# facebookresearch/spdl

Hardware: AMD Instinct MI355X
Metric: images/sec device-resident JPEG→RGB224, 1/2/4/8×MI355X; % HBM roofline (higher is better)
Workload: dtype u8; 1 GPU; configs[1]: synthetic 480x640 q90 4:2:0 baseline JPEG resident in HBM -> RGB 224x224 u8 (scale bicubic decrease + centred pad, rgb24); global_batch=256, per_gpu_batch=256, distinct_images=32, lanes=4, hw_queues=4, entropy_threads=256, entropy_piece_bytes=131072

## Files before the change

### spdl_amd/csrc/hj_common.h

```cpp
#pragma once
#include <stddef.h>
#include <stdint.h>

#ifndef HJ_HD
#define HJ_HD __host__ __device__
#endif

namespace hj {

constexpr int kMaxComp = 4;

enum { kColorGray = 0, kColorYcbcr, kColorRgb, kColorCmyk, kColorYcck, kColorYcbcrk };
inline HJ_HD bool frame_color(int ncomp, const int32_t* h, const int32_t* v, const int* ids,
                              int adobe, int32_t* color) {
  bool all11 = true;
  for (int c = 0; c < ncomp; c++) all11 = all11 && h[c] == 1 && v[c] == 1;
  if (ncomp == 1) {
    *color = kColorGray;
  } else if (ncomp == 3) {
    const bool rgb = adobe == 0 || (ids[0] == 'R' && ids[1] == 'G' && ids[2] == 'B');
    if (rgb && !all11) return false;
    *color = rgb ? kColorRgb : kColorYcbcr;
  } else {
    if (!all11) return false;
// ... 159 lines not shown
};
inline HJ_HD IdctDivMod idct_divmod(uint32_t n, uint32_t d, uint32_t magic) {
  uint32_t q = (uint32_t)(((uint64_t)n * magic) >> 32);
  uint32_t r = n - q * d;
  if (r >= d) {
    q += 1;
    r -= d;
  }
  return {q, r};
}
struct IdctBlockPos {
  int c, bx, by;
};
inline HJ_HD IdctBlockPos idct_block_pos(const ImageInfo& in, uint32_t j) {
  const IdctDivMod m = idct_divmod(j, (uint32_t)in.bpm, in.bpm_magic);
  const IdctDivMod p = idct_divmod(m.q, (uint32_t)in.mcux, in.mcux_magic);
  const int b = (int)m.r, c = in.mcu_comp[b];
  if (in.ncomp == 1) return {c, (int)p.r, (int)p.q};
  return {c, (int)p.r * in.comp_h[c] + in.mcu_dx[b], (int)p.q * in.comp_v[c] + in.mcu_dy[b]};
}

inline HJ_HD uint32_t idct_region_block(const ImageInfo& in, int mx0, int my0, int mw,
                                        uint32_t mw_magic, uint32_t l) {
  const IdctDivMod m = idct_divmod(l, (uint32_t)in.bpm, in.bpm_magic);
  const IdctDivMod p = idct_divmod(m.q, (uint32_t)mw, mw_magic);
  return ((uint32_t)(my0 + (int)p.q) * (uint32_t)in.mcux + (uint32_t)(mx0 + (int)p.r)) *
             (uint32_t)in.bpm + m.r;
}

constexpr int kDsChunk = 4096;
constexpr int kIdctThreads = 256;
constexpr int kHsRows = 16;
struct DsChunk {
  int32_t keep, rst, term;
  int32_t keep_pre, rst_pre;
  int32_t pad_[3];
};

struct SwsCsc {
  int32_t crv, cbu, cgu, cgv;
  int32_t y_coeff, y_offset, v2r, v2g, u2g, u2b;
};

#ifndef HJ_ABLATIONS
#define HJ_ABLATIONS 0
#endif
enum Ablate : int32_t {
  kAblSwsHpass = 0x100,
  kAblSwsVpass = 0x200,
  kAblSwsStore = 0x400,
  kAblIdctNone = 0x800,
  kAblEntWrite = 0x1000,
  kAblEntSync = 0x2000,
  kAblEntList = 0x4000,
  kAblEntDc = 0x8000,
  kAblEntDesc = 0x80000,
  kAblEntropy = kAblEntWrite | kAblEntSync | kAblEntList | kAblEntDc | kAblEntDesc,
  kAblNoMultiscan = 0x10000,
  kAblNoIdct = 0x20000,
  kAblNoOutput = 0x40000,
};

struct BatchParams {
  int32_t n;
  int32_t pix_fmt, dtype, idct;
  int32_t resize, filter;
  int32_t out_w, out_h;
  int32_t sub_bits;
  int32_t debug_mask;
// ... 31 lines not shown
```

### spdl_amd/csrc/hj_destuff.h

```cpp
#pragma once
#include <cstdint>

#ifndef HJ_HD
#define HJ_HD __host__ __device__
#endif

namespace hj {

HJ_HD inline int ds_ctz(uint32_t v) {
#if defined(__HIP_DEVICE_COMPILE__)
  return __ffs((int)v) - 1;
#else
  return __builtin_ctz(v);
#endif
}
HJ_HD inline int ds_top(uint32_t v) {
#if defined(__HIP_DEVICE_COMPILE__)
  return 31 - __clz((int)v);
#else
  return 31 - __builtin_clz(v);
#endif
}
HJ_HD inline int ds_popc(uint32_t v) {
#if defined(__HIP_DEVICE_COMPILE__)
// ... 140 lines not shown
    }
  }
}

HJ_HD inline void ds_compact_begin(uint32_t (&w)[4], uint32_t keep, uint32_t& drop) {
#pragma unroll
  for (int i = 0; i < 4; i++) {
    const uint32_t m = (((keep >> (4 * i)) & 15u) * 0x204081u) & 0x01010101u;
    w[i] &= ds_perm(0u, 0u, 0x0C0C0C0Cu + m);
  }
  drop = keep ? ~keep & ((1u << ds_top(keep)) - 1u) & ~((1u << ds_ctz(keep)) - 1u) : 0u;
}

HJ_HD inline void ds_compact_step(uint32_t (&w)[4], uint32_t& drop) {
  const int p = ds_ctz(drop | 0x10000u);
  drop = (drop >> 1) & (0xFFFFFFFFu << p);
  const uint32_t up = 0xFFFF0000u >> (16 - p);
#pragma unroll
  for (int i = 0; i < 4; i++) {
    const uint32_t inc = (((up >> (4 * i)) & 15u) * 0x204081u) & 0x01010101u;
    w[i] = ds_perm(i < 3 ? w[i + 1] : 0u, w[i], 0x03020100u + inc);
  }
}

HJ_HD inline void ds_shift_words(const uint32_t (&w)[4], uint32_t s, uint32_t (&x)[5]) {
  const uint32_t sel = 0x07060504u - ds_perm(0u, s, 0u);
  x[0] = ds_perm(w[0], 0u, sel);
  x[1] = ds_perm(w[1], w[0], sel);
  x[2] = ds_perm(w[2], w[1], sel);
  x[3] = ds_perm(w[3], w[2], sel);
  x[4] = ds_perm(0u, w[3], sel);
}

}
```

### spdl_amd/csrc/hj_kernels.hip

```cpp
#include <hip/hip_fp16.h>
#include <hip/hip_runtime.h>

#include "hj_common.h"
#include "hj_destuff.h"
#include "hj_idct.h"
#include "hj_launch.h"
#include "hj_sws_tile.h"
#include "hj_upsample.h"

namespace hj {

__device__ __forceinline__ uint32_t rfl(uint32_t v) { return __builtin_amdgcn_readfirstlane(v); }


struct ParseScratch {
  ImageInfo info;
  uint16_t qt[4][64];
  uint8_t bits[8][17];
  uint8_t vals[8][256];
  int32_t have[8];
  int32_t qhave[4];
  int32_t maxcode[8][18];
  int32_t valoff[8][17];
  int32_t dqt_off[4], dqt_pq[4];
// ... 177 lines not shown
          for (int y = 0; y < in.comp_v[c]; y++)
            for (int x = 0; x < in.comp_h[c]; x++) {
              if (b >= kMaxBpm) return kErrUnsupported;
              in.mcu_comp[b] = c;
              in.mcu_dx[b] = x;
              in.mcu_dy[b] = y;
              b++;
            }
        }
        in.bpm = b;
      }
      in.nblocks = in.mcux * in.mcuy * in.bpm;
      in.bpm_magic = idct_div_magic((uint32_t)in.bpm);
      in.mcux_magic = idct_div_magic((uint32_t)in.mcux);
      return kOk;
    }
  }
}

__global__ void __launch_bounds__(256, 8) parse_kernel(const uint8_t* __restrict__ bytes,
                                                    const ImageDesc* __restrict__ host_desc,
                                                    ImageDesc* __restrict__ desc,
                                                    ImageInfo* __restrict__ infos,
                                                    HuffTable* __restrict__ luts,
                                                    const uint4* __restrict__ host_tables,
                                                    uint4* __restrict__ tables, int64_t ntab16,
                                                    const uint32_t* __restrict__ host_work,
                                                    uint32_t* __restrict__ work, int nwork,
                                                    uint64_t* __restrict__ chain,
                                                    uint32_t* __restrict__ ds_map,
                                                    uint32_t* __restrict__ idct_map,
                                                    uint32_t* __restrict__ hs_map,
                                                    uint32_t* __restrict__ sws_map,
                                                    const int ndesc) {
  __shared__ ParseScratch s;
  __shared__ int st;
  __shared__ __attribute__((aligned(16))) uint8_t hdr[kHdrBytes];
  const int img = blockIdx.x, tid = threadIdx.x;
#if HJ_PARSE_PROF
  int64_t pt[8];
  int npt = 0;
  pt[npt++] = wall_clock64();
#define HJ_PT() (pt[npt++] = wall_clock64())
#else
#define HJ_PT() ((void)0)
#endif
  __shared__ __attribute__((aligned(16))) ImageDesc sdd;
  {
    static_assert(sizeof(ImageDesc) % 8 == 0, "descriptor copied in 8-byte words");
    const uint64_t* src = reinterpret_cast<const uint64_t*>((host_desc ? host_desc : desc) + img);
    uint64_t* dst = reinterpret_cast<uint64_t*>(desc + img);
    uint64_t* sdst = reinterpret_cast<uint64_t*>(&sdd);
    for (int i = tid; i < (int)(sizeof(ImageDesc) / 8); i += blockDim.x) {
      const uint64_t v = src[i];
      if (host_desc) dst[i] = v;
      sdst[i] = v;
    }
  }
  if (host_desc) {
    for (int64_t i = (int64_t)img * blockDim.x + tid; i < ntab16;
         i += (int64_t)gridDim.x * blockDim.x)
      tables[i] = host_tables[i];
    for (int i = img * blockDim.x + tid; i < nwork; i += gridDim.x * blockDim.x)
      work[i] = host_work[i];
  }
  for (int v = (int)gridDim.x + img; v < ndesc; v += (int)gridDim.x) {
    const ImageDesc* sv = (host_desc ? host_desc : desc) + v;
    if (host_desc) {
      const uint64_t* src = reinterpret_cast<const uint64_t*>(sv);
      uint64_t* dst = reinterpret_cast<uint64_t*>(desc + v);
      for (int i = tid; i < (int)(sizeof(ImageDesc) / 8); i += blockDim.x) dst[i] = src[i];
    }
    const int hs0 = sv->hs_wg0, hsn = sv->hs_wgs, sw0 = sv->sws_wg0,
              swn = sv->sws_bands * sv->sws_chunks;
    for (int i = tid; i < hsn; i += blockDim.x) hs_map[hs0 + i] = (uint32_t)v;
    for (int i = tid; i < swn; i += blockDim.x) sws_map[sw0 + i] = (uint32_t)v;
  }
  __syncthreads();
  const ImageDesc& dd = sdd;
  for (int i = tid; i < dd.ds_cap; i += blockDim.x) ds_map[dd.ds_wg0 + i] = (uint32_t)img;
  for (int i = tid; i < (dd.idct_blocks + kIdctThreads - 1) / kIdctThreads; i += blockDim.x)
    idct_map[dd.idct_wg0 + i] = (uint32_t)img;
  for (int i = tid; i < dd.hs_wgs; i += blockDim.x) hs_map[dd.hs_wg0 + i] = (uint32_t)img;
  for (int i = tid; i < dd.sws_bands * dd.sws_chunks; i += blockDim.x)
    sws_map[dd.sws_wg0 + i] = (uint32_t)img;
  if (img == 0 && tid == 0) chain[0] = 0ull;
  if (dd.pieces > 1)
    for (int i = tid; i < dd.pieces * kChainGranules; i += blockDim.x)
      chain[kChainHead + dd.chain_off + i] = 0ull;
  {
    int* z = reinterpret_cast<int*>(&s);
    for (int i = tid; i < (int)(sizeof(ParseScratch) / 4); i += blockDim.x) z[i] = 0;
  }
  const int nh = (int)min(dd.in_size, (int64_t)kHdrBytes) & ~15;
  for (int i = tid; i < nh / 16; i += blockDim.x)
    reinterpret_cast<uint4*>(hdr)[i] = reinterpret_cast<const uint4*>(bytes + dd.in_off)[i];
  __syncthreads();
  HJ_PT();
  if (tid == 0) {
    const Bytes file{bytes + dd.in_off, (lds_u8*)hdr, nh};
    int rc = parse_headers(file, (int)dd.in_size, s);
    if (rc == kOk) {
      if (s.info.width != dd.width || s.info.height != dd.height || s.info.ncomp != dd.ncomp ||
          s.info.nblocks != dd.nblocks || s.info.color != dd.color)
        rc = kErrBadHeader;
      for (int c = 0; c < s.info.ncomp && rc == kOk; c++)
        if (s.info.comp_h[c] != dd.h_samp[c] || s.info.comp_v[c] != dd.v_samp[c])
          rc = kErrBadHeader;
      if (rc == kOk && s.info.ri > 0 &&
          (s.info.mcux * s.info.mcuy + s.info.ri - 1) / s.info.ri > dd.seg_cap)
        rc = kErrBadRestart;
    }
    if (rc == kOk && dd.refuse) rc = dd.refuse;
// ... 84 lines not shown
    tab_nsub[t] = nsub;
  }
  __syncthreads();
  if (tid == 0) {
    int ns = 0, seen = 0, subs = 0, slow = 0;
    for (int c = 0; c < s.info.ncomp; c++)
      for (int k = 0; k < 2; k++) {
        const int slot = k == 0 ? s.info.dc_tab[c] : 4 + s.info.ac_tab[c];
        if (!(seen & (1 << slot))) {
          ns++;
          subs += tab_nsub[slot];
          slow |= (tab_slow >> slot) & 1;
          slow |= tab_nsub[slot] > (kSubShare >> kSubBits);
        }
        seen |= 1 << slot;
      }
    s.info.ent_wide = !(ns <= 4 && (subs << kSubBits) <= kSubPool && !slow);
  }
  __syncthreads();
  HJ_PT();
#if HJ_PARSE_PROF
  if (tid == 0)
    for (int i = 1; i < npt && i < 8; i++) s.info.sdiag[39 + i] = (int32_t)(pt[i] - pt[0]);
#endif
  static_assert(sizeof(ImageInfo) % 4 == 0, "ImageInfo copied in words");
  {
    const uint32_t* src = reinterpret_cast<const uint32_t*>(&s.info);
    uint32_t* dst = reinterpret_cast<uint32_t*>(infos + img);
    for (int i = tid; i < (int)(sizeof(ImageInfo) / 4); i += blockDim.x) dst[i] = src[i];
  }
}


__global__ void __launch_bounds__(256) lut_kernel(const uint8_t* __restrict__ bytes,
                                                  const ImageDesc* __restrict__ desc,
                                                  ImageInfo* __restrict__ infos,
                                                  HuffTable* __restrict__ luts) {
  __shared__ int first, same, maxcode[18], valoff[17];
  __shared__ uint8_t bits[17], vals[256];
  const int t = blockIdx.x, img = blockIdx.y, tid = threadIdx.x;
  const ImageInfo& in = infos[img];
  if (in.status != kOk || in.multiscan || in.tab_n[t] == 0) return;
  const uint32_t h = in.tab_hash[t];
  const int n = in.tab_n[t];
  const uint8_t* d = bytes + desc[img].in_off + in.tab_off[t];
  if (tid == 0) first = img;
  __syncthreads();
  for (int j = tid; j < img; j += blockDim.x) {
    const ImageInfo& o = infos[j];
    if (o.status == kOk && !o.multiscan && o.tab_n[t] == n && o.tab_hash[t] == h)
      atomicMin(&first, j);
  }
  __syncthreads();
  const int j = first;
  if (j < img) {
    if (tid == 0) same = 1;
    __syncthreads();
    const uint8_t* e = bytes + desc[j].in_off + infos[j].tab_off[t];
    for (int k = tid; k < 16 + n; k += blockDim.x)
      if (d[k] != e[k]) same = 0;
    __syncthreads();
    if (same) {
      if (tid == 0) infos[img].lut_ref[t] = j * 8 + t;
      return;
    }
  }
  if (tid < 16) bits[tid + 1] = d[tid];
  for (int k = tid; k < 256; k += blockDim.x) vals[k] = k < n ? d[16 + k] : 0;
  __syncthreads();
  if (tid == 0) {
    int code = 0, k = 0;
    for (int l = 1; l <= 16; l++) {
      if (bits[l]) {
        valoff[l] = k - code;
        code += bits[l];
        k += bits[l];
        maxcode[l] = code - 1;
      } else {
        maxcode[l] = -1;
        valoff[l] = 0;
      }
      code <<= 1;
    }
    maxcode[17] = 0x7FFFFFFF;
// ... 22 lines not shown
          if (sz) {
            const int raw = (int)((w16 >> (16 - l - sz)) & ((1u << sz) - 1));
            v = raw < (1 << (sz - 1)) ? raw - ((1 << sz) - 1) : raw;
          }
          return hj_entry(kKindFull, l + sz, sym, is_dc, v);
        }
        return hj_entry(kKindCode, l, sym, is_dc, 0);
      }
    }
    return 0u;
  };
  for (int idx = tid; idx < kLutSize; idx += blockDim.x) {
    uint32_t e = entry16((uint32_t)idx << kSubBits, kLutBits, kLutBits);
    if (e == 0u && idx >= p_lo && idx <= p_hi)
      e = sub_ok ? ((kKindSub << 5) | ((uint32_t)(idx - p_lo) << kEntHiShift)) : 0u;
    T.lut[idx] = e ? e : 1u;
  }
  if (sub_ok)
    for (int i = tid; i < nsub << kSubBits; i += blockDim.x)
      T.sub[i] = max(entry16(((uint32_t)(p_lo + (i >> kSubBits)) << kSubBits) |
                                 (uint32_t)(i & ((1 << kSubBits) - 1)),
                             16, 16),
                     1u);
  if (tid == 0) {
    T.nsub = sub_ok ? nsub : 0;
    T.long_slow = sub_ok ? 0 : 1;
    T.sub_lo = sub_ok ? p_lo : 0;
  }
  if (tid < 18) T.maxcode[tid] = maxcode[tid];
  if (tid < 17) T.valoff[tid] = valoff[tid];
  for (int i = tid; i < 256; i += blockDim.x) T.vals[i] = vals[i];
}


constexpr int kDsThreads = 256;
constexpr int kDsPer = kDsChunk / kDsThreads;

__device__ __forceinline__ int wave_incl_scan(int v) {
  const int lane = threadIdx.x & 63;
#pragma unroll
  for (int d = 1; d < 64; d <<= 1) {
    const int u = __shfl_up(v, d, 64);
    if (lane >= d) v += u;
  }
  return v;
}

__device__ __forceinline__ void wg_scan2(int a, int b, int& ea, int& eb, int& ta, int& tb,
                                        int* sh ) {
  const int lane = threadIdx.x & 63, wid = threadIdx.x >> 6;
  const int ia = wave_incl_scan(a), ib = wave_incl_scan(b);
  if (lane == 63) {
    sh[wid] = ia;
    sh[4 + wid] = ib;
  }
  __syncthreads();
  ea = ia - a;
  eb = ib - b;
  ta = tb = 0;
#pragma unroll
  for (int w = 0; w < 4; w++) {
    if (w < wid) {
      ea += sh[w];
      eb += sh[4 + w];
    }
    ta += sh[w];
    tb += sh[4 + w];
  }
}

__device__ __forceinline__ int wave_incl_scan_dpp(int v) {
  v += __builtin_amdgcn_update_dpp(0, v, 0x111, 0xF, 0xF, false);
  v += __builtin_amdgcn_update_dpp(0, v, 0x112, 0xF, 0xF, false);
  v += __builtin_amdgcn_update_dpp(0, v, 0x114, 0xF, 0xF, false);
  v += __builtin_amdgcn_update_dpp(0, v, 0x118, 0xF, 0xF, false);
  v += __builtin_amdgcn_update_dpp(0, v, 0x142, 0xA, 0xF, false);
  v += __builtin_amdgcn_update_dpp(0, v, 0x143, 0xC, 0xF, false);
  return v;
}

__device__ __forceinline__ void wg_scan1(int v, int& ex, int& tot, int* sh ) {
  const int lane = threadIdx.x & 63, wid = threadIdx.x >> 6;
  const int iv = wave_incl_scan_dpp(v);
  if (lane == 63) sh[wid] = iv;
  __syncthreads();
  ex = iv - v;
  tot = 0;
#pragma unroll
  for (int w = 0; w < 4; w++) {
    if (w < wid) ex += sh[w];
    tot += sh[w];
  }
}

__device__ __forceinline__ void ds_load(const uint8_t* __restrict__ d, int size, int j0,
                                        uint32_t (&w)[4], uint32_t& prev, uint32_t& next) {
  prev = ds_prev_byte(d, size, j0);
  if (j0 + 16 <= size) {
    const uint4 q = *reinterpret_cast<const uint4*>(d + j0);
    w[0] = q.x;
    w[1] = q.y;
    w[2] = q.z;
    w[3] = q.w;
  } else {
    ds_load_bytes(d, size, j0, w);
  }
  next = ds_next_byte(d, size, j0);
}

constexpr int kDsStageWords = (16 + 16 + kDsChunk + 32) / 4;

__device__ __forceinline__ void stage_to_global(uint8_t* __restrict__ dst, const uint32_t* stage,
                                                int n, int tid) {
  const int a = (int)((uintptr_t)dst & 15);
  const uint8_t* src = reinterpret_cast<const uint8_t*>(stage) + 16 + a;
  const int head = min(n, (16 - a) & 15);
  if (tid < head) dst[tid] = src[tid];
  const int nv = (n - head) >> 4;
  const uint4* s4 = reinterpret_cast<const uint4*>(src + head);
  uint4* d4 = reinterpret_cast<uint4*>(dst + head);
  for (int i = tid; i < nv; i += kDsThreads) d4[i] = s4[i];
  const int t0 = head + 16 * nv;
  if (t0 + tid < n) dst[t0 + tid] = src[t0 + tid];
}

__global__ void __launch_bounds__(kDsThreads) destuff_count_kernel(
    const uint8_t* __restrict__ bytes, const ImageDesc* __restrict__ desc,
    const ImageInfo* __restrict__ infos, DsChunk* __restrict__ chunks,
    const uint32_t* __restrict__ ds_map) {
  __shared__ int shsum, shterm;
  const bool flat = ds_map != nullptr;
  const int img = flat ? (int)ds_map[blockIdx.x] : (int)blockIdx.y;
  const int k = flat ? (int)blockIdx.x - desc[img].ds_wg0 : (int)blockIdx.x, tid = threadIdx.x;
  if (infos[img].status != kOk || infos[img].multiscan) return;
  const ImageDesc& dd = desc[img];
  const int size = (int)dd.in_size, start = infos[img].scan_start;
  const int cbase = (start & ~15) + k * kDsChunk;
  if (cbase >= size || k >= dd.ds_cap) return;
  if (tid == 0) {
    shsum = 0;
    shterm = 0x7FFFFFFF;
  }
  __syncthreads();
  const uint8_t* d = bytes + dd.in_off;
  const int j0 = cbase + tid * kDsPer;
  uint32_t w[4], prev, next;
  ds_load(d, size, j0, w, prev, next);
  uint32_t slow;
  int cnt = ds_count_words(w, prev, next, j0, start, size, slow);
  if (slow) {
    uint32_t rst;
    int term;
    ds_resolve(d, size, j0, slow, rst, term);
    cnt += __popc(rst) << 16;
    if (term != 0x7FFFFFFF) atomicMin(&shterm, term);
  }
  const int wsum = wave_incl_scan_dpp(cnt);
  if ((tid & 63) == 63) atomicAdd(&shsum, wsum);
  __syncthreads();
  if (tid == 0) {
    DsChunk& c = chunks[dd.ds_off + k];
    c.keep = shsum & 0xFFFF;
    c.rst = shsum >> 16;
    c.term = shterm;
  }
}

__global__ void __launch_bounds__(kDsThreads) destuff_prefix_kernel(
    const ImageDesc* __restrict__ desc, ImageInfo* __restrict__ infos,
    DsChunk* __restrict__ chunks) {
  __shared__ int sh[8];
  __shared__ int shterm;
  const int img = blockIdx.x, tid = threadIdx.x;
  if (infos[img].status != kOk || infos[img].multiscan) return;
  const ImageDesc& dd = desc[img];
  const int size = (int)dd.in_size, start = infos[img].scan_start;
  const int base = start & ~15;
  const int nch = min(dd.ds_cap, (size - base + kDsChunk - 1) / kDsChunk);
  if (tid == 0) shterm = 0x7FFFFFFF;
  __syncthreads();
  for (int k = tid; k < nch; k += kDsThreads) atomicMin(&shterm, chunks[dd.ds_off + k].term);
  __syncthreads();
  const int end = min(shterm, size);
  int ck = 0, cr = 0;
  for (int k0 = 0; k0 < nch; k0 += kDsThreads) {
    const int k = k0 + tid;
    const bool v = k < nch && base + k * kDsChunk < end;
    const int kk = v ? chunks[dd.ds_off + k].keep : 0, rr = v ? chunks[dd.ds_off + k].rst : 0;
    int ek, er, tk, tr;
    wg_scan2(kk, rr, ek, er, tk, tr, sh);
    if (k < nch) {
      chunks[dd.ds_off + k].keep_pre = ck + ek;
      chunks[dd.ds_off + k].rst_pre = cr + er;
    }
    ck += tk;
    cr += tr;
    __syncthreads();
  }
  if (tid == 0) infos[img].scan_end = end;
}

__global__ void __launch_bounds__(kDsThreads) destuff_write_kernel(
    const uint8_t* __restrict__ bytes, const ImageDesc* __restrict__ desc,
    ImageInfo* __restrict__ infos, const DsChunk* __restrict__ chunks, uint8_t* __restrict__ clean,
    uint32_t* __restrict__ segs, const uint32_t* __restrict__ ds_map) {
  __shared__ int sh[4];
  __shared__ __attribute__((aligned(16))) uint32_t stage[kDsStageWords];
  const bool flat = ds_map != nullptr;
  const int img = flat ? (int)ds_map[blockIdx.x] : (int)blockIdx.y;
  const int k = flat ? (int)blockIdx.x - desc[img].ds_wg0 : (int)blockIdx.x, tid = threadIdx.x;
  if (infos[img].status != kOk || infos[img].multiscan) return;
  const ImageDesc& dd = desc[img];
  const int size = (int)dd.in_size, start = infos[img].scan_start, end = infos[img].scan_end;
  const int base = start & ~15;
  const int cbase = base + k * kDsChunk;
  const int last = (max(end - 1, start) - base) / kDsChunk;
  if (k > last || k >= dd.ds_cap) return;
  for (int i = tid; i < kDsStageWords / 4; i += kDsThreads)
    reinterpret_cast<uint4*>(stage)[i] = make_uint4(0, 0, 0, 0);
  const uint8_t* d = bytes + dd.in_off;
  const int j0 = cbase + tid * kDsPer;
  uint32_t w[4], prev, next;
  ds_load(d, size, j0, w, prev, next);
  const DsMasks m = ds_classify_words(w, prev, next, j0, start, end);
  const uint32_t keep = m.keep;
  uint32_t rst = 0;
  if (m.slow) {
    int term;
    ds_resolve(d, size, j0, m.slow, rst, term);
  }
  int ex, tot;
  wg_scan1((int)(__popc(rst) << 16 | __popc(keep)), ex, tot, sh);
  const int ek = ex & 0xFFFF, er = ex >> 16, tk = tot & 0xFFFF, tr = tot >> 16;
  const DsChunk& c = chunks[dd.ds_off + k];
  uint32_t* sg = segs + dd.seg_off;
  if (rst) {
    int r = c.rst_pre + er;
    bool overflow = false;
    for (uint32_t q = rst; q; q &= q - 1) {
      const int i = ds_ctz(q);
      r++;
      if (r < dd.seg_cap) sg[r] = (uint32_t)(c.keep_pre + ek + __popc(keep & ((1u << i) - 1u)));
      else overflow = true;
    }
    if (overflow) infos[img].status = kErrBadRestart;
  }
  uint8_t* out = clean + dd.in_off + c.keep_pre;
  uint32_t drop;
  ds_compact_begin(w, keep, drop);
  while (__any(drop != 0u)) ds_compact_step(w, drop);
  if (keep) {
    const int p = 16 + (int)((uintptr_t)out & 15) + ek - ds_ctz(keep);
    uint32_t x[5];
    ds_shift_words(w, (uint32_t)(p & 3), x);
    uint32_t* q = stage + (p >> 2);
#pragma unroll
    for (int i = 0; i < 5; i++) atomicOr(q + i, x[i]);
  }
  __syncthreads();
  stage_to_global(out, stage, tk, tid);
  if (k == last) {
    const int clen = c.keep_pre + tk;
    if (tid < 64) out[tk + tid] = 0;
    if (tid == 0) {
      infos[img].clean_len = clen;
      infos[img].nseg = min(c.rst_pre + tr + 1, dd.seg_cap);
      sg[0] = 0;
    }
  }
}


constexpr int kMaxTabs = 2 * kMaxComp;
__constant__ uint8_t kSlotOrder[64] = {
    0,  4,  8,  16, 12, 1,  5,  9,  20, 24, 32, 28, 17, 13, 2,  6,  10, 21, 25, 36, 40, 48,
    44, 33, 29, 18, 14, 3,  7,  11, 22, 26, 37, 41, 52, 56, 60, 49, 45, 34, 30, 19, 15, 23,
    27, 38, 42, 53, 57, 61, 50, 46, 35, 31, 39, 43, 54, 58, 62, 51, 47, 55, 59, 63};
constexpr int kWinWords = 12;

template <int NT, int NTAB>
struct EntShared {
  static constexpr int kTabs = NTAB;
  uint32_t lut[NTAB][kLutSize];
  uint32_t sub[kSubPool];
  int32_t maxcode[NTAB][18];
  int32_t valoff[NTAB][17];
  uint8_t vals[NTAB][256];
  uint32_t run_pos[NT];
  uint32_t run_zb[NT];
  uint32_t qdc[kMaxComp];
  union {
    uint32_t win[kWinWords][NT];
    struct {
      int32_t scan_flag[NT];
      int32_t scan_v[NT][kMaxComp];
      int32_t red[NT];
    } sc;
  };
  int32_t flag;
// ... 387 lines not shown
    done = (bad && past_a) || stop || (trunc && past_b);
    rc = (bad && !past_a) ? kErrBadHuffman : ((trunc && !past_b) ? kErrTruncated : kOk);
    const bool bend = zn >= 64u;
    if (bend && !stop && o.open) close_block(o, nb - 1);
    const uint32_t bsn = hot_next(m, d.bs);
    d.z = bend ? 0u : zn;
    d.bs = bend ? bsn : d.bs;
  }
  if (o.open && d.z != 0u) close_block(o, nb - 1);
  hot_flip(m, d);
  return rc;
}

template <int NT, int NV, class SH>
__device__ void seg_scan(SH& S, int tid, int flag, const int (&v)[kMaxComp]) {
  S.sc.scan_flag[tid] = flag;
#pragma unroll
  for (int i = 0; i < NV; i++) S.sc.scan_v[tid][i] = v[i];
  __syncthreads();
  for (int off = 1; off < NT; off <<= 1) {
    int pf = 0, pv[NV];
    const bool take = tid >= off;
#pragma unroll
    for (int i = 0; i < NV; i++) pv[i] = take ? S.sc.scan_v[tid - off][i] : 0;
    if (take) pf = S.sc.scan_flag[tid - off];
    __syncthreads();
    if (take && !S.sc.scan_flag[tid]) {
#pragma unroll
      for (int i = 0; i < NV; i++) S.sc.scan_v[tid][i] += pv[i];
      S.sc.scan_flag[tid] = pf;
    }
    __syncthreads();
  }
}

typedef __attribute__((address_space(1))) unsigned long long hj_gu64;
__device__ __forceinline__ void gran_put(uint64_t* c, int i, uint32_t tag, uint32_t v) {
  __hip_atomic_store((hj_gu64*)(c + i), ((unsigned long long)tag << 32) | v, __ATOMIC_RELAXED,
                     __HIP_MEMORY_SCOPE_AGENT);
}
__device__ __forceinline__ uint64_t gran_get(const uint64_t* c, int i) {
  return __hip_atomic_load((hj_gu64*)(c + i), __ATOMIC_RELAXED, __HIP_MEMORY_SCOPE_AGENT);
}
constexpr int64_t kPollGapTicks = 100000;
struct WaitBound {
  int64_t last, idle;
  int sig;
};
__device__ __forceinline__ WaitBound wait_begin() { return WaitBound{wall_clock64(), 0, -1}; }
__device__ __forceinline__ bool wait_expired(WaitBound& w, int sig, int64_t limit) {
  const int64_t now = wall_clock64(), dt = now - w.last;
  w.last = now;
  if (sig != w.sig) {
    w.sig = sig;
    w.idle = 0;
    return false;
  }
  if (dt < kPollGapTicks) w.idle += dt;
  return w.idle >= limit;
}

__device__ __forceinline__ void chain_fail(uint64_t* rec, int tid) {
  if (tid < kChainGranules) gran_put(rec, tid, kTagFail, 0u);
}

template <class SH>
__device__ void chain_lookback(SH& S, const uint64_t* chain, int p, int lane, int64_t limit) {
  const uint64_t* rec = chain + (int64_t)(p - 1 - lane) * kChainGranules;
  const bool mine = lane < p;
  WaitBound wb = wait_begin();
  for (;;) {
    uint64_t r[8] = {};
    if (mine) {
#pragma unroll
      for (int i = 0; i < 8; i++) r[i] = gran_get(rec, i);
    }
    bool fail = false, has1 = mine, has2 = mine;
    int present = 0;
#pragma unroll
    for (int i = 0; i < 8; i++) {
      const uint32_t tag = (uint32_t)(r[i] >> 32);
      fail |= tag == kTagFail;
      present += __popcll(__ballot(tag != 0u));
      if (i < 5) has1 = has1 && tag == kTagRec1;
      else has2 = has2 && tag == kTagRec2;
    }
    if (__any(fail)) {
      if (lane == 0) S.lb_ok = -1;
      return;
    }
    const uint64_t m2 = __ballot(has2), m1 = __ballot(has1);
    if (m2 != 0) {
// ... 4331 lines not shown
      hmax = max(hmax, dd.h_samp[c]);
      vmax = max(vmax, dd.v_samp[c]);
    }
  }
  int v[3][2][8];
#pragma unroll
  for (int c = 0; c < 3; c++) {
    if (c < dd.ncomp) {
      const int hr = dd.ncomp > 1 ? hmax / dd.h_samp[c] : 1;
      const int vr = dd.ncomp > 1 ? vmax / dd.v_samp[c] : 1;
      const int cw = dd.win_w[c], ch = dd.win_h[c];
      up::run8x2(planes + dd.plane_off[c], dd.plane_stride[c], cw, ch, up::mode_of(hr, vr, cw), hr,
                 vr, x0, y0, v[c][0], v[c][1]);
    } else {
#pragma unroll
      for (int k = 0; k < 8; k++) {
        v[c][0][k] = v[0][0][k];
        v[c][1][k] = v[0][1][k];
      }
    }
  }
  turbo_row(out, dd, p, x0, y0, v[0][0], v[1][0], v[2][0]);
  if (y0 + 1 < H) turbo_row(out, dd, p, x0, y0 + 1, v[0][1], v[1][1], v[2][1]);
}


hipError_t launch_parse(const BatchBuffers& b, const ImageDesc* host_desc, const void* host_tables,
                        int64_t table_bytes, int threads, hipStream_t st) {
  const auto* host_work =
      host_desc ? reinterpret_cast<const uint32_t*>(host_desc + b.ndesc) : nullptr;
  hipLaunchKernelGGL(parse_kernel, dim3(b.n), dim3(threads), 0, st, b.bytes, host_desc, b.desc,
                     b.infos, b.luts, static_cast<const uint4*>(host_tables),
                     reinterpret_cast<uint4*>(b.wts), (table_bytes + 15) / 16, host_work, b.work,
                     b.nwork, b.chain, b.ds_map, b.idct_map, b.hs_map, b.sws_map, b.ndesc);
  hipLaunchKernelGGL(lut_kernel, dim3(8, b.n), dim3(256), 0, st, b.bytes, b.desc, b.infos, b.luts);
  return hipGetLastError();
}
hipError_t launch_destuff(const BatchBuffers& b, bool flat, int ds_wgs, int max_chunks,
                          hipStream_t st) {
  const dim3 grid = flat ? dim3(ds_wgs) : dim3(max_chunks, b.n);
  const uint32_t* map = flat ? b.ds_map : nullptr;
  hipLaunchKernelGGL(destuff_count_kernel, grid, dim3(kDsThreads), 0, st, b.bytes, b.desc, b.infos,
                     b.dschunks, map);
  hipLaunchKernelGGL(destuff_prefix_kernel, dim3(b.n), dim3(kDsThreads), 0, st, b.desc, b.infos,
                     b.dschunks);
  hipLaunchKernelGGL(destuff_write_kernel, grid, dim3(kDsThreads), 0, st, b.bytes, b.desc, b.infos,
                     b.dschunks, b.clean, b.segs, map);
  return hipGetLastError();
}
hipError_t launch_entropy(const BatchBuffers& b, const EntropyParams& ep, int threads, int lds_pad,
                          hipStream_t st) {
#define HJ_ENT(T, NTAB)                                                                        \
  hipLaunchKernelGGL((entropy_kernel<T, NTAB>), dim3(b.nwork), dim3(T), lds_pad, st, b.clean,  \
                     b.segs, b.desc, b.infos, b.luts, b.ents, b.bdesc, b.recs, b.work, b.chain, \
                     ep, b.nwork)
  switch (threads) {
    case 1024: HJ_ENT(1024, 4); break;
    case 512: HJ_ENT(512, 4); break;
    case 128: HJ_ENT(128, 4); break;
    default: HJ_ENT(256, 4);
  }
#undef HJ_ENT
  return hipGetLastError();
}
hipError_t launch_multiscan(const BatchBuffers& b, hipStream_t st) {
  hipLaunchKernelGGL(multiscan_kernel, dim3(b.n), dim3(256), 0, st, b.bytes, b.clean, b.desc,
                     b.infos, b.ents, b.bdesc);
  return hipGetLastError();
}
#define HJ_IDCT_KIND(K, kind, ...)                               \
  do {                                                           \
    if ((kind) == 2) hipLaunchKernelGGL(K<2>, __VA_ARGS__);      \
    else if ((kind) == 1) hipLaunchKernelGGL(K<1>, __VA_ARGS__); \
    else hipLaunchKernelGGL(K<0>, __VA_ARGS__);                  \
  } while (0)
hipError_t launch_idct(const BatchBuffers& b, int idct, bool flat, int idct_wgs, int max_blocks,
                       int xcd, hipStream_t st) {
  const int max_tiles = (max_blocks + kIdctThreads - 1) / kIdctThreads;
  const dim3 grid = flat ? dim3(idct_wgs) : dim3(max_tiles, b.n);
  HJ_IDCT_KIND(idct_kernel, idct, grid, dim3(kIdctThreads), 0, st, b.ents, b.bdesc, b.desc, b.infos,
// ... 83 lines not shown
```

Baseline: 607,700 images/sec.

## Fuse three-pass destuff into single-pass decoupled lookback kernel with LUT build

Replaces the count/prefix/write destuff kernels with one kernel that publishes per-chunk aggregates and uses a decoupled lookback across prior chunks to get its output offset, so the input is read once and two launches disappear. The Huffman LUT build kernel is folded into the same launch as extra workgroups, and chunk records are zeroed in the parse kernel. This removes launch overhead and a second pass over the JPEG bytes, at the cost of spin-waiting on predecessors (with a timeout) and dropping the status/multiscan filter in LUT dedup.

```diff
diff --git a/spdl_amd/csrc/hj_common.h b/spdl_amd/csrc/hj_common.h
--- a/spdl_amd/csrc/hj_common.h
+++ b/spdl_amd/csrc/hj_common.h
@@ -215,9 +215,7 @@
 constexpr int kIdctThreads = 256;
 constexpr int kHsRows = 16;
 struct DsChunk {
-  int32_t keep, rst, term;
-  int32_t keep_pre, rst_pre;
-  int32_t pad_[3];
+  uint64_t rec;
 };
 
 struct SwsCsc {
diff --git a/spdl_amd/csrc/hj_destuff.h b/spdl_amd/csrc/hj_destuff.h
--- a/spdl_amd/csrc/hj_destuff.h
+++ b/spdl_amd/csrc/hj_destuff.h
@@ -196,4 +196,35 @@
   x[4] = ds_perm(0u, w[3], sel);
 }
 
-}
+enum DsState : uint32_t {
+  kDsNone = 0,
+  kDsOpen = 1,
+  kDsEnd = 2,
+  kDsFail = 3,
+};
+struct DsAgg {
+  int32_t keep, rst;
+  uint32_t state;
+};
+HJ_HD inline uint64_t ds_agg_pack(const DsAgg& a) {
+  return (uint64_t)a.state << 32 | (uint32_t)a.rst << 16 | (uint32_t)a.keep;
+}
+HJ_HD inline DsAgg ds_agg_unpack(uint64_t r) {
+  return DsAgg{(int32_t)(r & 0xFFFFu), (int32_t)((r >> 16) & 0xFFFFu), (uint32_t)(r >> 32)};
+}
+HJ_HD inline DsAgg ds_agg_combine(const DsAgg& a, const DsAgg& b) {
+  if (a.state != kDsOpen) return a;
+  return DsAgg{a.keep + b.keep, a.rst + b.rst, b.state};
+}
+HJ_HD inline uint32_t ds_cut_mask(int j0, int term) {
+  return term <= j0 ? 0u : term - j0 >= 16 ? 0xFFFFu : (1u << (term - j0)) - 1u;
+}
+HJ_HD inline bool ds_chunk_finishes(const DsAgg& pre, int term, int k, int last_chunk) {
+  return pre.state == kDsOpen && (term != 0x7FFFFFFF || k == last_chunk);
+}
+HJ_HD inline int ds_last_chunk(int start, int size, int chunk) {
+  const int lastb = size - 1 > start ? size - 1 : start;
+  return (lastb - (start & ~15)) / chunk;
+}
+
+}
diff --git a/spdl_amd/csrc/hj_kernels.hip b/spdl_amd/csrc/hj_kernels.hip
--- a/spdl_amd/csrc/hj_kernels.hip
+++ b/spdl_amd/csrc/hj_kernels.hip
@@ -233,6 +233,7 @@
                                                     uint32_t* __restrict__ idct_map,
                                                     uint32_t* __restrict__ hs_map,
                                                     uint32_t* __restrict__ sws_map,
+                                                    DsChunk* __restrict__ dschunks,
                                                     const int ndesc) {
   __shared__ ParseScratch s;
   __shared__ int st;
@@ -280,6 +281,7 @@
   __syncthreads();
   const ImageDesc& dd = sdd;
   for (int i = tid; i < dd.ds_cap; i += blockDim.x) ds_map[dd.ds_wg0 + i] = (uint32_t)img;
+  for (int i = tid; i < dd.ds_cap; i += blockDim.x) dschunks[dd.ds_off + i].rec = 0ull;
   for (int i = tid; i < (dd.idct_blocks + kIdctThreads - 1) / kIdctThreads; i += blockDim.x)
     idct_map[dd.idct_wg0 + i] = (uint32_t)img;
   for (int i = tid; i < dd.hs_wgs; i += blockDim.x) hs_map[dd.hs_wg0 + i] = (uint32_t)img;
@@ -430,15 +432,25 @@
 }
 
 
-__global__ void __launch_bounds__(256) lut_kernel(const uint8_t* __restrict__ bytes,
-                                                  const ImageDesc* __restrict__ desc,
-                                                  ImageInfo* __restrict__ infos,
-                                                  HuffTable* __restrict__ luts) {
-  __shared__ int first, same, maxcode[18], valoff[17];
-  __shared__ uint8_t bits[17], vals[256];
-  const int t = blockIdx.x, img = blockIdx.y, tid = threadIdx.x;
+struct LutScratch {
+  int first, same, maxcode[18], valoff[17];
+  uint8_t bits[17], vals[256];
+};
+
+__device__ __forceinline__ void lut_build(const uint8_t* __restrict__ bytes,
+                                          const ImageDesc* __restrict__ desc,
+                                          ImageInfo* __restrict__ infos,
+                                          HuffTable* __restrict__ luts, const int t, const int img,
+                                          LutScratch& L) {
+  int& first = L.first;
+  int& same = L.same;
+  int(&maxcode)[18] = L.maxcode;
+  int(&valoff)[17] = L.valoff;
+  uint8_t(&bits)[17] = L.bits;
+  uint8_t(&vals)[256] = L.vals;
+  const int tid = threadIdx.x;
   const ImageInfo& in = infos[img];
-  if (in.status != kOk || in.multiscan || in.tab_n[t] == 0) return;
+  if (in.tab_n[t] == 0) return;
   const uint32_t h = in.tab_hash[t];
   const int n = in.tab_n[t];
   const uint8_t* d = bytes + desc[img].in_off + in.tab_off[t];
@@ -446,8 +458,7 @@
   __syncthreads();
   for (int j = tid; j < img; j += blockDim.x) {
     const ImageInfo& o = infos[j];
-    if (o.status == kOk && !o.multiscan && o.tab_n[t] == n && o.tab_hash[t] == h)
-      atomicMin(&first, j);
+    if (o.tab_n[t] == n && o.tab_hash[t] == h) atomicMin(&first, j);
   }
   __syncthreads();
   const int j = first;
@@ -536,6 +547,32 @@
   for (int i = tid; i < 256; i += blockDim.x) T.vals[i] = vals[i];
 }
 
+typedef __attribute__((address_space(1))) unsigned long long hj_gu64;
+__device__ __forceinline__ void gran_put(uint64_t* c, int i, uint32_t tag, uint32_t v) {
+  __hip_atomic_store((hj_gu64*)(c + i), ((unsigned long long)tag << 32) | v, __ATOMIC_RELAXED,
+                     __HIP_MEMORY_SCOPE_AGENT);
+}
+__device__ __forceinline__ uint64_t gran_get(const uint64_t* c, int i) {
+  return __hip_atomic_load((hj_gu64*)(c + i), __ATOMIC_RELAXED, __HIP_MEMORY_SCOPE_AGENT);
+}
+constexpr int64_t kPollGapTicks = 100000;
+struct WaitBound {
+  int64_t last, idle;
+  int sig;
+};
+__device__ __forceinline__ WaitBound wait_begin() { return WaitBound{wall_clock64(), 0, -1}; }
+__device__ __forceinline__ bool wait_expired(WaitBound& w, int sig, int64_t limit) {
+  const int64_t now = wall_clock64(), dt = now - w.last;
+  w.last = now;
+  if (sig != w.sig) {
+    w.sig = sig;
+    w.idle = 0;
+    return false;
+  }
+  if (dt < kPollGapTicks) w.idle += dt;
+  return w.idle >= limit;
+}
+
 
 constexpr int kDsThreads = 256;
 constexpr int kDsPer = kDsChunk / kDsThreads;
@@ -548,29 +585,6 @@
     if (lane >= d) v += u;
   }
   return v;
-}
-
-__device__ __forceinline__ void wg_scan2(int a, int b, int& ea, int& eb, int& ta, int& tb,
-                                        int* sh ) {
-  const int lane = threadIdx.x & 63, wid = threadIdx.x >> 6;
-  const int ia = wave_incl_scan(a), ib = wave_incl_scan(b);
-  if (lane == 63) {
-    sh[wid] = ia;
-    sh[4 + wid] = ib;
-  }
-  __syncthreads();
-  ea = ia - a;
-  eb = ib - b;
-  ta = tb = 0;
-#pragma unroll
-  for (int w = 0; w < 4; w++) {
-    if (w < wid) {
-      ea += sh[w];
-      eb += sh[4 + w];
-    }
-    ta += sh[w];
-    tb += sh[4 + w];
-  }
 }
 
 __device__ __forceinline__ int wave_incl_scan_dpp(int v) {
@@ -581,20 +595,6 @@
   v += __builtin_amdgcn_update_dpp(0, v, 0x142, 0xA, 0xF, false);
   v += __builtin_amdgcn_update_dpp(0, v, 0x143, 0xC, 0xF, false);
   return v;
-}
-
-__device__ __forceinline__ void wg_scan1(int v, int& ex, int& tot, int* sh ) {
-  const int lane = threadIdx.x & 63, wid = threadIdx.x >> 6;
-  const int iv = wave_incl_scan_dpp(v);
-  if (lane == 63) sh[wid] = iv;
-  __syncthreads();
-  ex = iv - v;
-  tot = 0;
-#pragma unroll
-  for (int w = 0; w < 4; w++) {
-    if (w < wid) ex += sh[w];
-    tot += sh[w];
-  }
 }
 
 __device__ __forceinline__ void ds_load(const uint8_t* __restrict__ d, int size, int j0,
@@ -628,131 +628,142 @@
   if (t0 + tid < n) dst[t0 + tid] = src[t0 + tid];
 }
 
-__global__ void __launch_bounds__(kDsThreads) destuff_count_kernel(
+constexpr int64_t kDsWaitTicks = 200000000;
+__device__ __forceinline__ DsAgg ds_lookback(const DsChunk* __restrict__ recs, int k, int lane,
+                                             bool& expired) {
+  DsAgg acc{0, 0, kDsOpen};
+  expired = false;
+  WaitBound wb = wait_begin();
+  for (int w0 = 0; w0 < k && acc.state == kDsOpen; w0 += 64) {
+    const int j = w0 + lane;
+    const bool mine = j < k;
+    for (;;) {
+      const DsAgg a = mine ? ds_agg_unpack(gran_get(&recs[j].rec, 0)) : DsAgg{0, 0, kDsOpen};
+      const uint64_t have = __ballot(a.state != kDsNone);
+      const uint64_t stop = __ballot(a.state == kDsEnd || a.state == kDsFail);
+      const int e = stop ? __builtin_ctzll(stop) : 63;
+      const uint64_t upto = e == 63 ? ~0ull : (1ull << (e + 1)) - 1ull;
+      if ((~have & upto) == 0ull) {
+        const bool in = lane <= e;
+        const int sk = wave_incl_scan_dpp(in ? a.keep : 0), sr = wave_incl_scan_dpp(in ? a.rst : 0);
+        const DsAgg win{__builtin_amdgcn_readlane(sk, 63), __builtin_amdgcn_readlane(sr, 63),
+                        (uint32_t)__builtin_amdgcn_readlane((int)a.state, e)};
+        acc = ds_agg_combine(acc, win);
+        break;
+      }
+      if (wait_expired(wb, __popcll(have) + w0, kDsWaitTicks)) {
+        expired = true;
+        return DsAgg{0, 0, kDsFail};
+      }
+      __builtin_amdgcn_s_sleep(2);
+    }
+  }
+  return acc;
+}
+
+__global__ void __launch_bounds__(kDsThreads) destuff_kernel(
     const uint8_t* __restrict__ bytes, const ImageDesc* __restrict__ desc,
-    const ImageInfo* __restrict__ infos, DsChunk* __restrict__ chunks,
-    const uint32_t* __restrict__ ds_map) {
-  __shared__ int shsum, shterm;
+    ImageInfo* __restrict__ infos, DsChunk* __restrict__ chunks, uint8_t* __restrict__ clean,
+    uint32_t* __restrict__ segs, const uint32_t* __restrict__ ds_map, HuffTable* __restrict__ luts,
+    const int ds_wgs, const int n) {
+  __shared__ int sh[8], shpre[3];
+  __shared__ __attribute__((aligned(16))) uint32_t stage[kDsStageWords];
+  static_assert(sizeof(LutScratch) <= sizeof(stage), "lut_build's scratch lies in the stage");
   const bool flat = ds_map != nullptr;
+  const int tid = threadIdx.x;
+  if (flat ? (int)blockIdx.x >= ds_wgs : (int)blockIdx.y >= n) {
+    const int l = flat ? (int)blockIdx.x - ds_wgs
+                       : ((int)blockIdx.y - n) * (int)gridDim.x + (int)blockIdx.x;
+    if (l < 8 * n)
+      lut_build(bytes, desc, infos, luts, l & 7, l >> 3, *reinterpret_cast<LutScratch*>(stage));
+    return;
+  }
   const int img = flat ? (int)ds_map[blockIdx.x] : (int)blockIdx.y;
-  const int k = flat ? (int)blockIdx.x - desc[img].ds_wg0 : (int)blockIdx.x, tid = threadIdx.x;
-  if (infos[img].status != kOk || infos[img].multiscan) return;
+  const int k = flat ? (int)blockIdx.x - desc[img].ds_wg0 : (int)blockIdx.x;
   const ImageDesc& dd = desc[img];
-  const int size = (int)dd.in_size, start = infos[img].scan_start;
-  const int cbase = (start & ~15) + k * kDsChunk;
-  if (cbase >= size || k >= dd.ds_cap) return;
-  if (tid == 0) {
-    shsum = 0;
-    shterm = 0x7FFFFFFF;
-  }
+  if (infos[img].multiscan || k >= dd.ds_cap) return;
+  DsChunk* recs = chunks + dd.ds_off;
+  if (tid == 0) shpre[2] = infos[img].status;
   __syncthreads();
-  const uint8_t* d = bytes + dd.in_off;
-  const int j0 = cbase + tid * kDsPer;
-  uint32_t w[4], prev, next;
-  ds_load(d, size, j0, w, prev, next);
-  uint32_t slow;
-  int cnt = ds_count_words(w, prev, next, j0, start, size, slow);
-  if (slow) {
-    uint32_t rst;
-    int term;
-    ds_resolve(d, size, j0, slow, rst, term);
-    cnt += __popc(rst) << 16;
-    if (term != 0x7FFFFFFF) atomicMin(&shterm, term);
-  }
-  const int wsum = wave_incl_scan_dpp(cnt);
-  if ((tid & 63) == 63) atomicAdd(&shsum, wsum);
-  __syncthreads();
-  if (tid == 0) {
-    DsChunk& c = chunks[dd.ds_off + k];
-    c.keep = shsum & 0xFFFF;
-    c.rst = shsum >> 16;
-    c.term = shterm;
-  }
-}
-
-__global__ void __launch_bounds__(kDsThreads) destuff_prefix_kernel(
-    const ImageDesc* __restrict__ desc, ImageInfo* __restrict__ infos,
-    DsChunk* __restrict__ chunks) {
-  __shared__ int sh[8];
-  __shared__ int shterm;
-  const int img = blockIdx.x, tid = threadIdx.x;
-  if (infos[img].status != kOk || infos[img].multiscan) return;
-  const ImageDesc& dd = desc[img];
+  if (shpre[2] != kOk) {
+    if (tid == 0) gran_put(&recs[k].rec, 0, kDsFail, 0u);
+    return;
+  }
   const int size = (int)dd.in_size, start = infos[img].scan_start;
   const int base = start & ~15;
-  const int nch = min(dd.ds_cap, (size - base + kDsChunk - 1) / kDsChunk);
-  if (tid == 0) shterm = 0x7FFFFFFF;
-  __syncthreads();
-  for (int k = tid; k < nch; k += kDsThreads) atomicMin(&shterm, chunks[dd.ds_off + k].term);
-  __syncthreads();
-  const int end = min(shterm, size);
-  int ck = 0, cr = 0;
-  for (int k0 = 0; k0 < nch; k0 += kDsThreads) {
-    const int k = k0 + tid;
-    const bool v = k < nch && base + k * kDsChunk < end;
-    const int kk = v ? chunks[dd.ds_off + k].keep : 0, rr = v ? chunks[dd.ds_off + k].rst : 0;
-    int ek, er, tk, tr;
-    wg_scan2(kk, rr, ek, er, tk, tr, sh);
-    if (k < nch) {
-      chunks[dd.ds_off + k].keep_pre = ck + ek;
-      chunks[dd.ds_off + k].rst_pre = cr + er;
-    }
-    ck += tk;
-    cr += tr;
-    __syncthreads();
-  }
-  if (tid == 0) infos[img].scan_end = end;
-}
-
-__global__ void __launch_bounds__(kDsThreads) destuff_write_kernel(
-    const uint8_t* __restrict__ bytes, const ImageDesc* __restrict__ desc,
-    ImageInfo* __restrict__ infos, const DsChunk* __restrict__ chunks, uint8_t* __restrict__ clean,
-    uint32_t* __restrict__ segs, const uint32_t* __restrict__ ds_map) {
-  __shared__ int sh[4];
-  __shared__ __attribute__((aligned(16))) uint32_t stage[kDsStageWords];
-  const bool flat = ds_map != nullptr;
-  const int img = flat ? (int)ds_map[blockIdx.x] : (int)blockIdx.y;
-  const int k = flat ? (int)blockIdx.x - desc[img].ds_wg0 : (int)blockIdx.x, tid = threadIdx.x;
-  if (infos[img].status != kOk || infos[img].multiscan) return;
-  const ImageDesc& dd = desc[img];
-  const int size = (int)dd.in_size, start = infos[img].scan_start, end = infos[img].scan_end;
-  const int base = start & ~15;
   const int cbase = base + k * kDsChunk;
-  const int last = (max(end - 1, start) - base) / kDsChunk;
-  if (k > last || k >= dd.ds_cap) return;
+  if (cbase >= size) return;
   for (int i = tid; i < kDsStageWords / 4; i += kDsThreads)
     reinterpret_cast<uint4*>(stage)[i] = make_uint4(0, 0, 0, 0);
   const uint8_t* d = bytes + dd.in_off;
   const int j0 = cbase + tid * kDsPer;
   uint32_t w[4], prev, next;
   ds_load(d, size, j0, w, prev, next);
-  const DsMasks m = ds_classify_words(w, prev, next, j0, start, end);
-  const uint32_t keep = m.keep;
-  uint32_t rst = 0;
-  if (m.slow) {
-    int term;
-    ds_resolve(d, size, j0, m.slow, rst, term);
-  }
-  int ex, tot;
-  wg_scan1((int)(__popc(rst) << 16 | __popc(keep)), ex, tot, sh);
+  const DsMasks m = ds_classify_words(w, prev, next, j0, start, size);
+  uint32_t keep = m.keep, rst = 0;
+  int term = 0x7FFFFFFF;
+  if (m.slow) ds_resolve(d, size, j0, m.slow, rst, term);
+  if (__any(term != 0x7FFFFFFF)) {
+    for (int o = 32; o > 0; o >>= 1) term = min(term, __shfl_xor(term, o));
+    const uint32_t cut = ds_cut_mask(j0, term);
+    keep &= cut;
+    rst &= cut;
+  }
+  const int cnt = (int)(__popc(rst) << 16 | __popc(keep));
+  const int iv = wave_incl_scan_dpp(cnt);
+  const int lane = tid & 63, wid = tid >> 6;
+  if (lane == 63) {
+    sh[wid] = iv;
+    sh[4 + wid] = term;
+  }
+  __syncthreads();
+  int ex = iv - cnt, tot = 0, cterm = 0x7FFFFFFF;
+  bool dead = false;
+#pragma unroll
+  for (int v = 0; v < 4; v++) {
+    if (v == wid) dead = cterm != 0x7FFFFFFF;
+    if (cterm == 0x7FFFFFFF) {
+      if (v < wid) ex += sh[v];
+      tot += sh[v];
+    }
+    cterm = min(cterm, sh[4 + v]);
+  }
+  if (dead) keep = rst = 0u;
   const int ek = ex & 0xFFFF, er = ex >> 16, tk = tot & 0xFFFF, tr = tot >> 16;
-  const DsChunk& c = chunks[dd.ds_off + k];
+  if (wid == 0) {
+    if (tid == 0)
+      gran_put(&recs[k].rec, 0, cterm != 0x7FFFFFFF ? kDsEnd : kDsOpen, (uint32_t)tot);
+    bool expired;
+    const DsAgg pre = ds_lookback(recs, k, lane, expired);
+    if (tid == 0) {
+      if (expired) {
+        infos[img].status = kErrDevice;
+        gran_put(&recs[k].rec, 0, kDsFail, 0u);
+      }
+      shpre[0] = pre.keep;
+      shpre[1] = pre.rst;
+      shpre[2] = (int)pre.state;
+    }
+  }
+  uint32_t drop;
+  ds_compact_begin(w, keep, drop);
+  while (__any(drop != 0u)) ds_compact_step(w, drop);
+  __syncthreads();
+  const DsAgg pre{shpre[0], shpre[1], (uint32_t)shpre[2]};
+  if (pre.state != kDsOpen) return;
   uint32_t* sg = segs + dd.seg_off;
   if (rst) {
-    int r = c.rst_pre + er;
+    int r = pre.rst + er;
     bool overflow = false;
     for (uint32_t q = rst; q; q &= q - 1) {
       const int i = ds_ctz(q);
       r++;
-      if (r < dd.seg_cap) sg[r] = (uint32_t)(c.keep_pre + ek + __popc(keep & ((1u << i) - 1u)));
+      if (r < dd.seg_cap) sg[r] = (uint32_t)(pre.keep + ek + __popc(keep & ((1u << i) - 1u)));
       else overflow = true;
     }
     if (overflow) infos[img].status = kErrBadRestart;
   }
-  uint8_t* out = clean + dd.in_off + c.keep_pre;
-  uint32_t drop;
-  ds_compact_begin(w, keep, drop);
-  while (__any(drop != 0u)) ds_compact_step(w, drop);
+  uint8_t* out = clean + dd.in_off + pre.keep;
   if (keep) {
     const int p = 16 + (int)((uintptr_t)out & 15) + ek - ds_ctz(keep);
     uint32_t x[5];
@@ -763,12 +774,12 @@
   }
   __syncthreads();
   stage_to_global(out, stage, tk, tid);
-  if (k == last) {
-    const int clen = c.keep_pre + tk;
+  if (ds_chunk_finishes(pre, cterm, k, ds_last_chunk(start, size, kDsChunk))) {
     if (tid < 64) out[tk + tid] = 0;
     if (tid == 0) {
-      infos[img].clean_len = clen;
-      infos[img].nseg = min(c.rst_pre + tr + 1, dd.seg_cap);
+      infos[img].clean_len = pre.keep + tk;
+      infos[img].nseg = min(pre.rst + tr + 1, dd.seg_cap);
+      infos[img].scan_end = min(cterm, size);
       sg[0] = 0;
     }
   }
@@ -1222,32 +1233,6 @@
     }
     __syncthreads();
   }
-}
-
-typedef __attribute__((address_space(1))) unsigned long long hj_gu64;
-__device__ __forceinline__ void gran_put(uint64_t* c, int i, uint32_t tag, uint32_t v) {
-  __hip_atomic_store((hj_gu64*)(c + i), ((unsigned long long)tag << 32) | v, __ATOMIC_RELAXED,
-                     __HIP_MEMORY_SCOPE_AGENT);
-}
-__device__ __forceinline__ uint64_t gran_get(const uint64_t* c, int i) {
-  return __hip_atomic_load((hj_gu64*)(c + i), __ATOMIC_RELAXED, __HIP_MEMORY_SCOPE_AGENT);
-}
-constexpr int64_t kPollGapTicks = 100000;
-struct WaitBound {
-  int64_t last, idle;
-  int sig;
-};
-__device__ __forceinline__ WaitBound wait_begin() { return WaitBound{wall_clock64(), 0, -1}; }
-__device__ __forceinline__ bool wait_expired(WaitBound& w, int sig, int64_t limit) {
-  const int64_t now = wall_clock64(), dt = now - w.last;
-  w.last = now;
-  if (sig != w.sig) {
-    w.sig = sig;
-    w.idle = 0;
-    return false;
-  }
-  if (dt < kPollGapTicks) w.idle += dt;
-  return w.idle >= limit;
 }
 
 __device__ __forceinline__ void chain_fail(uint64_t* rec, int tid) {
@@ -5645,20 +5630,17 @@
   hipLaunchKernelGGL(parse_kernel, dim3(b.n), dim3(threads), 0, st, b.bytes, host_desc, b.desc,
                      b.infos, b.luts, static_cast<const uint4*>(host_tables),
                      reinterpret_cast<uint4*>(b.wts), (table_bytes + 15) / 16, host_work, b.work,
-                     b.nwork, b.chain, b.ds_map, b.idct_map, b.hs_map, b.sws_map, b.ndesc);
-  hipLaunchKernelGGL(lut_kernel, dim3(8, b.n), dim3(256), 0, st, b.bytes, b.desc, b.infos, b.luts);
+                     b.nwork, b.chain, b.ds_map, b.idct_map, b.hs_map, b.sws_map, b.dschunks,
+                     b.ndesc);
   return hipGetLastError();
 }
 hipError_t launch_destuff(const BatchBuffers& b, bool flat, int ds_wgs, int max_chunks,
                           hipStream_t st) {
-  const dim3 grid = flat ? dim3(ds_wgs) : dim3(max_chunks, b.n);
-  const uint32_t* map = flat ? b.ds_map : nullptr;
-  hipLaunchKernelGGL(destuff_count_kernel, grid, dim3(kDsThreads), 0, st, b.bytes, b.desc, b.infos,
-                     b.dschunks, map);
-  hipLaunchKernelGGL(destuff_prefix_kernel, dim3(b.n), dim3(kDsThreads), 0, st, b.desc, b.infos,
-                     b.dschunks);
-  hipLaunchKernelGGL(destuff_write_kernel, grid, dim3(kDsThreads), 0, st, b.bytes, b.desc, b.infos,
-                     b.dschunks, b.clean, b.segs, map);
+  const int lut_wgs = 8 * b.n;
+  const dim3 grid = flat ? dim3(ds_wgs + lut_wgs)
+                         : dim3(max_chunks, b.n + (lut_wgs + max_chunks - 1) / max_chunks);
+  hipLaunchKernelGGL(destuff_kernel, grid, dim3(kDsThreads), 0, st, b.bytes, b.desc, b.infos,
+                     b.dschunks, b.clean, b.segs, flat ? b.ds_map : nullptr, b.luts, ds_wgs, b.n);
   return hipGetLastError();
 }
 hipError_t launch_entropy(const BatchBuffers& b, const EntropyParams& ep, int threads, int lds_pad,
```

Result: slower. 594,400 images/sec (-2.2%).
